# apache/incubator-predictionio

Measured on NVIDIA H100. Metric: ALS iterations/sec, higher is better.
Workload: dtype f32

## Files before the change

incubator-predictionio_b200/csrc/als_lockstep.cuh:

```cuda
#pragma once
#include <cuda_runtime.h>
#include <stdint.h>

namespace pio {

template <int N>
struct LsLayout {
  static constexpr int NBK = N / 16;
  static constexpr int NOFF = NBK * (NBK - 1) / 2;
  static constexpr int DIAG0 = NOFF * 256;
  static constexpr int SIZE = DIAG0 + NBK * 136;
  static constexpr int STRIDE = SIZE + ((SIZE % 32) == 16 ? 0 : (48 - SIZE % 32) % 32);
  __host__ __device__ static constexpr int swz(int rr) { return ((rr >> 1) & 1) * 2 + ((rr >> 2) & 1); }
  __host__ __device__ static constexpr int offd_base(int rb, int cb) { return (rb * (rb - 1) / 2 + cb) * 256; }
  __host__ __device__ static constexpr int offd(int rb, int cb, int rr, int cc) {
    return offd_base(rb, cb) + rr * 16 + 4 * ((cc >> 2) ^ swz(rr)) + (cc & 3);
  }
  __host__ __device__ static constexpr int diag(int rb, int rr, int cc) { return DIAG0 + rb * 136 + rr * (rr + 1) / 2 + cc; }
  __host__ __device__ static constexpr int at(int r, int c) {
    return (r >> 4) == (c >> 4) ? diag(r >> 4, r & 15, c & 15) : offd(r >> 4, c >> 4, r & 15, c & 15);
  }
};

__device__ __forceinline__ float ls_rsqrt(float x) {
  float r;
  asm("rsqrt.approx.ftz.f32 %0, %1;" : "=f"(r) : "f"(x));
  return r;
}

template <int N>
__device__ __forceinline__ void ls_add_yty(float* __restrict__ slot, const float* __restrict__ yty) {
  using LL = LsLayout<N>;
  const int lane = threadIdx.x & 31;
  for (int o = lane; o < LL::NOFF * 64; o += 32) {
    const int b = o >> 6, rr = (o >> 2) & 15, cg = o & 3;
    int rb = 1;
    while (rb * (rb + 1) / 2 <= b) ++rb;
    const int cb = b - rb * (rb - 1) / 2;
    float4* d = reinterpret_cast<float4*>(slot + LL::offd_base(rb, cb) + rr * 16 + 4 * (cg ^ LL::swz(rr)));
    const float4 y = __ldg(reinterpret_cast<const float4*>(yty + (size_t)(16 * rb + rr) * N + 16 * cb + 4 * cg));
    float4 v = *d;
    v.x += y.x; v.y += y.y; v.z += y.z; v.w += y.w;
    *d = v;
  }
  for (int o = lane; o < LL::NBK * 256; o += 32) {
    const int rb = o >> 8, rr = (o >> 4) & 15, cc = o & 15;
    if (cc <= rr) slot[LL::diag(rb, rr, cc)] += __ldg(yty + (size_t)(16 * rb + rr) * N + 16 * rb + cc);
  }
}

template <int N>
__device__ __forceinline__ void chol_lockstep(float* __restrict__ slot, const float* __restrict__ bvec, float ridge, int k,
                                              float* __restrict__ colbuf, float* __restrict__ dst_row, bool valid,
                                              int* __restrict__ fail) {
  using LL = LsLayout<N>;
  constexpr int LANES = N / 4;
  constexpr int Q = LANES / 16;
  constexpr int NBK = N / 16;
  static_assert(N == 64 || N == 128, "lockstep solver: N = 64 (two matrices per warp) or 128 (one)");
  const int lane = threadIdx.x & 31;
  const int l = lane % LANES, lq = l >> 4, lr = l & 15;
  const int sw = LL::swz(lr);
  float bb[4], yv[4], dv[4];
#pragma unroll
  for (int i = 0; i < 4; ++i) {
    bb[i] = bvec[i * LANES + l];
    yv[i] = 0.f;
    dv[i] = 0.f;
  }
  bool bad = false;
  __syncwarp();

#pragma unroll
  for (int p = 0; p < NBK; ++p) {
    constexpr int dummy = 0;
    (void)dummy;
    const int sp = p / Q;
    const bool isdiag = (Q == 1) || (lq == (p % Q));
    float a[4][16];
#pragma unroll
    for (int i = 0; i < 4; ++i) {
      if (i < sp) continue;
      const int bi = i * Q + lq;
      const int r = i * LANES + l;
      if (i == sp) {
#pragma unroll
        for (int c = 0; c < 16; ++c) {
          float v = 0.f;
          if (bi == p) {
            if (c <= lr) v = slot[LL::diag(p, lr, c)];
          } else if (bi > p) {
            v = slot[LL::offd(bi, p, lr, c)];
          }
          a[i][c] = v;
        }
      } else {
        const float* rowp = slot + LL::offd_base(bi, p) + lr * 16;
#pragma unroll
        for (int cg = 0; cg < 4; ++cg) {
          const float4 v = *reinterpret_cast<const float4*>(rowp + 4 * (cg ^ sw));
          a[i][4 * cg + 0] = v.x; a[i][4 * cg + 1] = v.y; a[i][4 * cg + 2] = v.z; a[i][4 * cg + 3] = v.w;
        }
      }
      if (i == sp) {
#pragma unroll
        for (int c = 0; c < 16; ++c)
          if (bi == p && c == lr) a[i][c] += ridge + (r >= k ? 1.f : 0.f);
      }
    }
    if (p > 0) {
#pragma unroll 1
      for (int q = 0; q < p; ++q) {
        const float* dblk = slot + LL::offd_base(p, q);
        const float* own[4];
#pragma unroll
        for (int i = 0; i < 4; ++i) {
          int bi = i * Q + lq;
          if (bi < p) bi = p;
          own[i] = slot + LL::offd_base(bi, q) + lr * 16;
        }
#pragma unroll 1
        for (int tg = 0; tg < 4; ++tg) {
          float4 o[4];
#pragma unroll
          for (int i = 0; i < 4; ++i)
            if (i >= sp) o[i] = *reinterpret_cast<const float4*>(own[i] + 4 * (tg ^ sw));
#pragma unroll
          for (int c = 0; c < 16; ++c) {
            const float4 d = *reinterpret_cast<const float4*>(dblk + c * 16 + 4 * (tg ^ LL::swz(c)));
#pragma unroll
            for (int i = 0; i < 4; ++i) {
              if (i < sp) continue;
              float v = a[i][c];
              v = fmaf(-o[i].x, d.x, v);
              v = fmaf(-o[i].y, d.y, v);
              v = fmaf(-o[i].z, d.z, v);
              v = fmaf(-o[i].w, d.w, v);
              a[i][c] = v;
            }
          }
        }
      }
    }
#pragma unroll
    for (int j = 0; j < 16; ++j) {
      float* cb = colbuf + (j & 1) * 32;
      if (isdiag) {
        cb[lr] = a[sp][j];
        cb[16 + lr] = bb[sp];
      }
      __syncwarp();
      float col[16];
#pragma unroll
      for (int cg = j / 4; cg < 4; ++cg) {
        const float4 v = *reinterpret_cast<const float4*>(cb + 4 * cg);
        col[4 * cg + 0] = v.x; col[4 * cg + 1] = v.y; col[4 * cg + 2] = v.z; col[4 * cg + 3] = v.w;
      }
      const float bg = cb[16 + j];
      float d = col[j];
      if (!(d > 0.f)) { bad = true; d = 1.f; }
      float inv = ls_rsqrt(d);
      inv = inv * (1.5f - 0.5f * d * inv * inv);
      const float inv2 = inv * inv;
      const float z = inv2 * bg;
      if (isdiag && lr == j) {
        yv[sp] = bg * inv;
        dv[sp] = inv;
      }
#pragma unroll
      for (int i = 0; i < 4; ++i) {
        if (i < sp) continue;
        const float aj = a[i][j];
        const float w = aj * inv2;
        if (i == sp) {
          const int bi = i * Q + lq;
          if (bi > p || (bi == p && lr > j)) bb[i] = fmaf(-aj, z, bb[i]);
        } else {
          bb[i] = fmaf(-aj, z, bb[i]);
        }
        a[i][j] = aj * inv;
#pragma unroll
        for (int c = j + 1; c < 16; ++c) a[i][c] = fmaf(-w, col[c], a[i][c]);
      }
    }
#pragma unroll
    for (int i = 0; i < 4; ++i) {
      if (i < sp) continue;
      const int bi = i * Q + lq;
      if (i == sp) {
#pragma unroll
        for (int c = 0; c < 16; ++c) {
          if (bi == p) {
            if (c <= lr) slot[LL::diag(p, lr, c)] = a[i][c];
          } else if (bi > p) {
            slot[LL::offd(bi, p, lr, c)] = a[i][c];
          }
        }
      } else {
        float* rowp = slot + LL::offd_base(bi, p) + lr * 16;
#pragma unroll
        for (int cg = 0; cg < 4; ++cg)
          *reinterpret_cast<float4*>(rowp + 4 * (cg ^ sw)) =
              make_float4(a[i][4 * cg + 0], a[i][4 * cg + 1], a[i][4 * cg + 2], a[i][4 * cg + 3]);
      }
    }
    __syncwarp();
  }

  float xs[4] = {0.f, 0.f, 0.f, 0.f};
#pragma unroll
  for (int g = N - 1; g >= 0; --g) {
    const int sg = g / LANES, lg = g % LANES, gb = g >> 4, gr = g & 15;
    const float t = yv[sg] * dv[sg];
    const float xg = __shfl_sync(0xffffffffu, t, lg, LANES);
    if (l == lg) xs[sg] = xg;
#pragma unroll
    for (int i = 0; i < 4; ++i) {
      if (i * Q > gb) continue;
      const int bi = i * Q + lq;
      if (bi < gb) yv[i] = fmaf(-slot[LL::offd(gb, bi, gr, lr)], xg, yv[i]);
      else if (bi == gb && lr < gr) yv[i] = fmaf(-slot[LL::diag(gb, gr, lr)], xg, yv[i]);
    }
  }
  if (valid) {
#pragma unroll
    for (int i = 0; i < 4; ++i) dst_row[i * LANES + l] = xs[i];
    if (bad && l == 0) atomicAdd(fail, 1);
  }
}

}
```

incubator-predictionio_b200/csrc/pio_als.cu:

```cuda
#include "../../include/pio_als.h"

#include <cuda_runtime.h>
#include <dlfcn.h>
#include <math.h>
#include <nccl.h>
#include <stdarg.h>
#include <stdio.h>
#include <stdlib.h>
#include <string.h>

#include <chrono>
#include <algorithm>
#include <array>
#include <deque>
#include <exception>
#include <map>
#include <mutex>
#include <string>
#include <type_traits>
#include <vector>

#include "als_kernels.cuh"
#include "als_mma_kernel.cuh"
#include "als_pair_kernel.cuh"
// ... 628 lines not shown
};
static int exchange_events(pio_als_handle* h, Scratch& keep, SortBufs& sb, long long n, XArr* arrs, int na,
                           long long* n_out) {
  cudaStream_t st = h->stream;
  NcclApi& nc = nccl_api();
  const int W = h->cfg.world_size, me = h->cfg.world_rank;
  Scratch tmp(h->stream);
  if (n > 0) CK(h, radix_sort_pairs(sb, (size_t)n, ceil_log2((uint64_t)W), st, &h->st.kernel_launches));
  const uint64_t* ks = sb.keys();
  const uint32_t* vs = sb.vals();
  long long *d_off = nullptr, *d_cnt = nullptr, *d_all = nullptr;
  CK(h, tmp.alloc(&d_off, (size_t)W + 1));
  CK(h, tmp.alloc(&d_cnt, (size_t)W));
  CK(h, tmp.alloc(&d_all, (size_t)W * W));
  CK(h, cudaMemsetAsync(d_off, 0, sizeof(long long) * (W + 1), st));
  if (n > 0) {
    build_ptr_kernel<<<nblk(n, 256), 256, 0, st>>>(ks, n, 0, W, d_off);
    LAUNCHED(h);
  }
  std::vector<long long> off(W + 1), all((size_t)W * W);
  CK(h, cudaMemcpyAsync(off.data(), d_off, sizeof(long long) * (W + 1), cudaMemcpyDeviceToHost, st));
  CK(h, cudaStreamSynchronize(st));
  std::vector<long long> cnt(W);
  for (int p = 0; p < W; ++p) cnt[p] = off[p + 1] - off[p];
  CK(h, cudaMemcpyAsync(d_cnt, cnt.data(), sizeof(long long) * W, cudaMemcpyHostToDevice, st));
  if (nc.AllGather(d_cnt, d_all, (size_t)W, ncclInt64, h->comm, st) != ncclSuccess)
    return fail(h, PIO_ALS_ERR_COMM, "ncclAllGather (exchange counts) failed");
  CK(h, cudaMemcpyAsync(all.data(), d_all, sizeof(long long) * W * W, cudaMemcpyDeviceToHost, st));
  CK(h, cudaStreamSynchronize(st));
  tmark(h, "  exchange: sort by rank + counts");
  std::vector<long long> roff(W + 1, 0);
  for (int src = 0; src < W; ++src) roff[src + 1] = roff[src] + all[(size_t)src * W + me];
  const long long nrecv = roff[W];
  if (nrecv >= (1ll << 32)) return fail(h, PIO_ALS_ERR_ARG, "more than 2^32-1 events on one rank after the exchange");
  std::vector<unsigned char*> sendbufs(na, nullptr), recvbufs(na, nullptr);
  for (int a = 0; a < na; ++a) {
    if (!arrs[a].in) { *arrs[a].out = nullptr; continue; }
    CK(h, tmp.alloc(&sendbufs[a], (size_t)(n > 0 ? n : 1) * arrs[a].elem));
    CK(h, keep.alloc(&recvbufs[a], (size_t)(nrecv > 0 ? nrecv : 1) * arrs[a].elem));
    if (n > 0) {
      if (arrs[a].elem == 4)
        gather_by_index_kernel<uint32_t><<<nblk(n, 256), 256, 0, st>>>((const uint32_t*)arrs[a].in, vs, n, (uint32_t*)sendbufs[a]);
      else
        gather_by_index_kernel<uint64_t><<<nblk(n, 256), 256, 0, st>>>((const uint64_t*)arrs[a].in, vs, n, (uint64_t*)sendbufs[a]);
      LAUNCHED(h);
    }
    *arrs[a].out = recvbufs[a];
  }
  if (nc.GroupStart() != ncclSuccess) return fail(h, PIO_ALS_ERR_COMM, "ncclGroupStart failed");
  for (int a = 0; a < na; ++a) {
    if (!arrs[a].in) continue;
    for (int p = 0; p < W; ++p) {
      const long long sc = cnt[p], rc_ = all[(size_t)p * W + me];
      if (sc > 0 && nc.Send(sendbufs[a] + (size_t)off[p] * arrs[a].elem, (size_t)sc * arrs[a].elem, ncclInt8, p, h->comm, st) != ncclSuccess)
        return fail(h, PIO_ALS_ERR_COMM, "ncclSend failed");
      if (rc_ > 0 && nc.Recv(recvbufs[a] + (size_t)roff[p] * arrs[a].elem, (size_t)rc_ * arrs[a].elem, ncclInt8, p, h->comm, st) != ncclSuccess)
        return fail(h, PIO_ALS_ERR_COMM, "ncclRecv failed");
    }
  }
  if (nc.GroupEnd() != ncclSuccess) return fail(h, PIO_ALS_ERR_COMM, "ncclGroupEnd failed");
  CK(h, cudaStreamSynchronize(st));
  tmark(h, "  exchange: gather + send/recv");
  *n_out = nrecv;
  return PIO_ALS_OK;
}

static int ingest_device(pio_als_handle* h, const int* d_user, const int* d_item, const float* d_rating,
                         long long nnz, int dedup, const long long* d_ts, bool sharded) {
  cudaStream_t st = h->stream;
  const int W = h->cfg.world_size;
  sharded = sharded && W > 1;
  if (nnz <= 0 && !sharded)
    return fail(h, PIO_ALS_ERR_ARG, "ratings cannot be empty (the templates require(!ratings.take(1).isEmpty))");
  if (nnz < 0) return fail(h, PIO_ALS_ERR_ARG, "nnz < 0");
  if (nnz >= (1ll << 32)) return fail(h, PIO_ALS_ERR_ARG, "nnz must be < 2^32 per call");
  if (dedup < 0 || dedup > 2) return fail(h, PIO_ALS_ERR_ARG, "bad dedup_mode %d", dedup);
  free_side(h, h->U, true);
  free_side(h, h->I, true);
  h->have_ratings = false;
  Side& U = h->U;
  Side& I = h->I;
  U.n = h->cfg.n_users;
  I.n = h->cfg.n_items;
  U.R = (U.n + W - 1) / W;
  I.R = (I.n + W - 1) / W;
  U.n_internal = U.R * W;
  I.n_internal = I.R * W;
  U.bits = ceil_log2((uint64_t)U.n_internal);
  I.bits = ceil_log2((uint64_t)I.n_internal);

  h->trace_on = getenv("PIO_ALS_INGEST_TRACE") != nullptr;
  h->t_prev = std::chrono::steady_clock::now();
  auto mark = [&](const char* what) { tmark(h, what); };
  CK(h, cudaMemsetAsync(h->d_fail, 0, sizeof(int), st));
  if (nnz > 0) {
    validate_coo_kernel<<<nblk(nnz, 256), 256, 0, st>>>(d_user, d_item, nnz, U.n, I.n, h->d_fail);
    LAUNCHED(h);
  }
  int bad = 0;
  CK(h, cudaMemcpyAsync(&bad, h->d_fail, sizeof(int), cudaMemcpyDeviceToHost, st));
  CK(h, cudaStreamSynchronize(st));
  if (bad) return fail(h, PIO_ALS_ERR_ARG, "%d ratings have a user/item index out of range", bad);

  mark("validate");
  Scratch tmp(h->stream);
  const int* su = d_user;
  const int* si = d_item;
  const float* sr = d_rating;
  const long long* sts = d_ts;
  long long ns = nnz;
  if (sharded && dedup != PIO_ALS_DEDUP_NONE) {
    Scratch xs(h->stream);
    SortBufs sb;
    for (int i : {0, 1}) {
      CK(h, xs.alloc(&sb.k[i], (size_t)nnz));
      CK(h, xs.alloc(&sb.v[i], (size_t)nnz));
    }
    if (nnz > 0) {
      dest_mod_kernel<<<nblk(nnz, 256), 256, 0, st>>>(d_user, nnz, W, sb.keys(), sb.vals());
      LAUNCHED(h);
    }
    void *xu = nullptr, *xi = nullptr, *xr = nullptr, *xt = nullptr;
    XArr arrs[4] = {{d_user, &xu, 4}, {d_item, &xi, 4}, {d_rating, &xr, 4},
                    {dedup == PIO_ALS_DEDUP_KEEP_LAST ? (const void*)d_ts : nullptr, &xt, 8}};
    int rc = exchange_events(h, tmp, sb, nnz, arrs, 4, &ns);
    if (rc) return rc;
    su = (const int*)xu; si = (const int*)xi; sr = (const float*)xr; sts = (const long long*)xt;
  }

  mark("exchange by user residue");
  const int* cu = su;
  const int* ci = si;
  const float* cr = sr;
  long long n2 = ns;
  if (dedup != PIO_ALS_DEDUP_NONE && ns > 0) {
    Scratch ds(h->stream);
    SortBufs sb;
    for (int i : {0, 1}) {
      CK(h, ds.alloc(&sb.k[i], (size_t)ns));
      CK(h, ds.alloc(&sb.v[i], (size_t)ns));
    }
    const int bu = ceil_log2((uint64_t)U.n), bi = ceil_log2((uint64_t)I.n);
    make_keys_ext_kernel<<<nblk(ns, 256), 256, 0, st>>>(su, si, ns, bi, sb.keys(), sb.vals());
    LAUNCHED(h);
    CK(h, radix_sort_pairs(sb, (size_t)ns, bu + bi, st, &h->st.kernel_launches));
    const uint64_t* ks = sb.keys();
    const uint32_t* vs = sb.vals();
    uint32_t* flag = nullptr;
    CK(h, ds.alloc(&flag, (size_t)ns));
    head_flags_kernel<<<nblk(ns, 256), 256, 0, st>>>(ks, ns, flag);
    LAUNCHED(h);
    uint32_t last_flag = 0, last_pos = 0;
    CK(h, cudaMemcpyAsync(&last_flag, flag + ns - 1, sizeof(uint32_t), cudaMemcpyDeviceToHost, st));
    CK(h, scan_exclusive_u32(flag, flag, (size_t)ns, st, &h->st.kernel_launches));
    CK(h, cudaMemcpyAsync(&last_pos, flag + ns - 1, sizeof(uint32_t), cudaMemcpyDeviceToHost, st));
    CK(h, cudaStreamSynchronize(st));
    n2 = (long long)last_pos + last_flag;
    int *du_ = nullptr, *di_ = nullptr;
    float* dr_ = nullptr;
    CK(h, tmp.alloc(&du_, (size_t)n2));
    CK(h, tmp.alloc(&di_, (size_t)n2));
    CK(h, tmp.alloc(&dr_, (size_t)n2));
    dedup_compact_kernel<<<nblk(ns, 256), 256, 0, st>>>(ks, vs, flag, ns, bi, sr, sts, dedup, du_, di_, dr_);
    LAUNCHED(h);
    cu = du_;
    ci = di_;
    cr = dr_;
  }

  mark("dedup");
  for (Side* s : {&U, &I}) {
    CK(h, dalloc(h, &s->deg, (size_t)s->n));
    CK(h, dalloc(h, &s->npos, (size_t)s->n));
    CK(h, dalloc(h, &s->perm, (size_t)s->n));
    CK(h, dalloc(h, &s->inv, (size_t)s->n_internal));
    CK(h, dalloc(h, &s->rpos, (size_t)s->n));
    CK(h, dalloc(h, &s->p2i, (size_t)s->n));
    CK(h, cudaMemsetAsync(s->deg, 0, sizeof(uint32_t) * s->n, st));
    CK(h, cudaMemsetAsync(s->npos, 0, sizeof(uint32_t) * s->n, st));
  }
  if (n2 > 0) {
    degree_kernel<<<nblk(n2, 256), 256, 0, st>>>(cu, ci, cr, n2, U.deg, I.deg, U.npos, I.npos);
    LAUNCHED(h);
  }
  CK(h, cudaMemsetAsync(h->d_absmax + 1, 0, sizeof(unsigned), st));
  if (n2 > 0) {
    pr::abs_max_kernel<<<std::min(nblk(n2, 256), 4u * h->sm_count), 256, 0, st>>>(cr, n2, h->d_absmax + 1);
    LAUNCHED(h);
  }
  long long n2_global = n2;
  if (sharded) {
    NcclApi& nc = nccl_api();
    long long* d_n = nullptr;
    CK(h, tmp.alloc(&d_n, 1));
    CK(h, cudaMemcpyAsync(d_n, &n2, sizeof(long long), cudaMemcpyHostToDevice, st));
    if (nc.GroupStart() != ncclSuccess) return fail(h, PIO_ALS_ERR_COMM, "ncclGroupStart failed");
    for (Side* s : {&U, &I}) {
      if (nc.AllReduce(s->deg, s->deg, (size_t)s->n, ncclUint32, ncclSum, h->comm, st) != ncclSuccess ||
          nc.AllReduce(s->npos, s->npos, (size_t)s->n, ncclUint32, ncclSum, h->comm, st) != ncclSuccess)
        return fail(h, PIO_ALS_ERR_COMM, "ncclAllReduce (degrees) failed");
    }
    if (nc.AllReduce(d_n, d_n, 1, ncclInt64, ncclSum, h->comm, st) != ncclSuccess ||
        nc.AllReduce(h->d_absmax + 1, h->d_absmax + 1, 1, ncclUint32, ncclMax, h->comm, st) != ncclSuccess)
      return fail(h, PIO_ALS_ERR_COMM, "ncclAllReduce (nnz, rating maximum) failed");
    if (nc.GroupEnd() != ncclSuccess) return fail(h, PIO_ALS_ERR_COMM, "ncclGroupEnd failed");
    CK(h, cudaMemcpyAsync(&n2_global, d_n, sizeof(long long), cudaMemcpyDeviceToHost, st));
    CK(h, cudaStreamSynchronize(st));
    if (n2_global <= 0)
      return fail(h, PIO_ALS_ERR_ARG, "ratings cannot be empty (the templates require(!ratings.take(1).isEmpty))");
  }
  h->st.nnz = n2_global;

  mark("degrees (+ all-reduce)");
  int rc = rank_rows(h, U);
  if (rc) return rc;
  rc = rank_rows(h, I);
  if (rc) return rc;

  mark("rank rows");
  if (!sharded) {
    rc = build_side(h, U, I, cu, ci, cr, n2, n2_global);
    if (rc) return rc;
    mark("build user side");
    rc = build_side(h, I, U, ci, cu, cr, n2, n2_global);
    if (rc) return rc;
    mark("build item side");
  } else {
    struct { Side* row; Side* col; const int* rowext; const int* colext; } jobs[2] = {{&U, &I, cu, ci}, {&I, &U, ci, cu}};
    for (auto& j : jobs) {
      Scratch xs(h->stream), recv(h->stream);
      SortBufs sb;
      for (int i : {0, 1}) {
        CK(h, xs.alloc(&sb.k[i], (size_t)n2));
        CK(h, xs.alloc(&sb.v[i], (size_t)n2));
      }
      if (n2 > 0) {
        dest_owner_kernel<<<nblk(n2, 256), 256, 0, st>>>(j.rowext, n2, j.row->perm, j.row->R, sb.keys(), sb.vals());
        LAUNCHED(h);
      }
      void *xrow = nullptr, *xcol = nullptr, *xr = nullptr;
      XArr arrs[3] = {{j.rowext, &xrow, 4}, {j.colext, &xcol, 4}, {cr, &xr, 4}};
      long long ne = 0;
      rc = exchange_events(h, recv, sb, n2, arrs, 3, &ne);
      if (rc) return rc;
      mark("exchange by row owner");
      rc = build_side(h, *j.row, *j.col, (const int*)xrow, (const int*)xcol, (const float*)xr, ne, n2_global);
      if (rc) return rc;
      mark("build side");
    }
  }

  for (Side* s : {&U, &I}) {
    if (!s->F) {
      CK(h, dalloc(h, &s->F, (size_t)s->n_internal * h->KP));
      h->have_init = false;
    }
    CK(h, dalloc(h, &s->cand_ext, (size_t)s->n_internal));
    cand_ext_kernel<<<nblk(s->n_internal, 256), 256, 0, st>>>(s->inv, s->deg, s->n_internal, s->cand_ext);
    LAUNCHED(h);
  }
  h->have_init = false;
  CK(h, cudaStreamSynchronize(st));
  mark("factor buffers");
  h->st.n_users_active = U.n_active;
  h->st.n_items_active = I.n_active;
  if (W > 1) {
    h->st.n_users_active = -1;
    h->st.n_items_active = -1;
  }
  h->have_ratings = true;
  h->trained = false;
  return PIO_ALS_OK;
}

static int init_hash(pio_als_handle* h) {
  cudaStream_t st = h->stream;
  CK(h, cudaMemsetAsync(h->U.F, 0, sizeof(float) * (size_t)h->U.n_internal * h->KP, st));
  CK(h, cudaMemsetAsync(h->I.F, 0, sizeof(float) * (size_t)h->I.n_internal * h->KP, st));
  hash_init_kernel<<<nblk(h->U.n, 128), 128, 0, st>>>(h->U.n, h->cfg.rank, h->KP, (uint64_t)h->cfg.seed, 0, h->U.perm,
                                                      h->U.deg, h->U.F);
  LAUNCHED(h);
  hash_init_kernel<<<nblk(h->I.n, 128), 128, 0, st>>>(h->I.n, h->cfg.rank, h->KP, (uint64_t)h->cfg.seed, 1, h->I.perm,
                                                      h->I.deg, h->I.F);
  LAUNCHED(h);
  h->have_init = true;
  return PIO_ALS_OK;
}

using Cfg16 = SolveCfg<16, 4, 25, 8>;
using Cfg32 = SolveCfg<32, 8, 25, 4>;
using Cfg64 = SolveCfg<64, 8, 7, 8>;
using Cfg128 = SolveCfg<128, 8, 2, 9>;

static_assert(fp32_rows_per_cta(16) == Cfg16::NG && fp32_rows_per_cta(32) == Cfg32::NG &&
              fp32_rows_per_cta(64) == Cfg64::NG && fp32_rows_per_cta(128) == Cfg128::NG, "SolveCfg::NG");
static_assert(Cfg16::WARP_CHOL && Cfg32::WARP_CHOL && Cfg64::WARP_CHOL && Cfg128::LS_PARTIAL,
              "als_finish_kernel runs one warp per row below KP 128, and KP 128 takes the LS128 route");
static_assert(MMA_ROWS_PER_CTA == mm::WARPS, "mm::WARPS");
static_assert(TC_ROWS_PER_CTA == tc::Api::kPerCta && TC_SOLVE_ROWS_PER_CTA == tc::Api::kSolveWarps, "tc::Api");
static_assert(LS128_FINISH_ROWS_PER_CTA == FIN128_WARPS, "FIN128_WARPS");
static_assert(PART % Cfg16::CH == 0 && PART % Cfg32::CH == 0 && PART % Cfg64::CH == 0 && PART % Cfg128::CH == 0 &&
              PART % mm::CH == 0 && PART % tc::STAGE_RATINGS == 0, "PART");
static_assert(PAIR_PART % pr::CH == 0 && pr::CH == 8, "PAIR_PART and PIO_ALS_PART round to multiples of pr::CH");

static int ensure_dyn_smem(pio_als_handle* h, const void* kernel, size_t bytes, bool carveout = false) {
  struct Rec {
    size_t bytes = 0;
    bool carveout = false;
  };
  static std::mutex mu;
  static std::map<std::pair<const void*, int>, Rec> recs;
  std::lock_guard<std::mutex> lk(mu);
  Rec& r = recs[std::make_pair(kernel, h->cfg.device)];
  if (r.bytes < bytes) {
    CK(h, cudaFuncSetAttribute(kernel, cudaFuncAttributeMaxDynamicSharedMemorySize, (int)bytes));
    r.bytes = bytes;
  }
  if (carveout && !r.carveout) {
    CK(h, cudaFuncSetAttribute(kernel, cudaFuncAttributePreferredSharedMemoryCarveout, 100));
    r.carveout = true;
  }
  return PIO_ALS_OK;
}

template <typename... KArgs, typename... Args>
static int solve_launch(pio_als_handle* h, void (*kernel)(KArgs...), int grid, int block, size_t smem, bool carveout,
                        cudaStream_t st, Args... args) {
  const int rc = ensure_dyn_smem(h, (const void*)kernel, smem, carveout);
  if (rc) return rc;
  kernel<<<grid, block, smem, st>>>(args...);
  LAUNCHED(h);
  ++h->st.solve_launches;
  CK(h, cudaGetLastError());
  return PIO_ALS_OK;
}

static void (*pair_kernel(int warps, bool imp))(const SolveParams, int) {
  switch (warps) {
    case 1: return imp ? pr::als_solve_pair_kernel<true, 1> : pr::als_solve_pair_kernel<false, 1>;
    case 2: return imp ? pr::als_solve_pair_kernel<true, 2> : pr::als_solve_pair_kernel<false, 2>;
    case 6: return imp ? pr::als_solve_pair_kernel<true, 6> : pr::als_solve_pair_kernel<false, 6>;
    case 12: return imp ? pr::als_solve_pair_kernel<true, 12> : pr::als_solve_pair_kernel<false, 12>;
    default: return imp ? pr::als_solve_pair_kernel<true, 4> : pr::als_solve_pair_kernel<false, 4>;
  }
}

static int tc_buffers(pio_als_handle* h, const Side& dst, tc::Api::Params* tp) {
  using A = tc::Api;
  tp->dbg = nullptr;
  tp->timing = nullptr;
  tp->out = nullptr;
  tp->out_row0 = 0;
  if (h->sw.tc_timing) {
    if (!h->d_timing) CK(h, cudaMalloc((void**)&h->d_timing, (size_t)h->sm_count * 16 * 8 * sizeof(long long)));
    cudaMemsetAsync(h->d_timing, 0, (size_t)h->sm_count * 16 * 8 * sizeof(long long), h->stream);
    tp->timing = h->d_timing;
  }
  if (h->sw.tc_debug) {
    if (h->dbg_rows < (size_t)dst.R) {
      if (h->d_dbg) cudaFree(h->d_dbg);
      CK(h, cudaMalloc((void**)&h->d_dbg, (size_t)dst.R * A::kRowFloats * sizeof(float)));
      h->dbg_rows = dst.R;
    }
    cudaMemsetAsync(h->d_dbg, 0, (size_t)dst.R * A::kRowFloats * sizeof(float), h->stream);
    tp->dbg = h->d_dbg;
  }
  if (h->sw.tc_split) {
    const int nlight = dst.n_active - dst.n_heavy;
    const size_t need = (size_t)(nlight < TC_TILE_ROWS ? nlight : TC_TILE_ROWS);
    if (h->tc_out_rows < need) {
      if (h->tc_out) cudaFree(h->tc_out);
      h->tc_out = nullptr;
      h->tc_out_rows = 0;
      CK(h, cudaMalloc((void**)&h->tc_out, need * A::kRowFloats * sizeof(float)));
      h->tc_out_rows = need;
    }
  }
  return PIO_ALS_OK;
}

template <class Cfg>
static int launch_solve_cfg(pio_als_handle* h, Side& dst, const Side& src) {
  SolveParams p0;
  p0.ptr = dst.ptr;
  p0.idx = dst.idx;
  p0.val = dst.val;
  p0.src = src.F;
  p0.dst = dst.F;
  p0.yty = h->yty;
  p0.nreg = dst.nreg;
  p0.fail = h->d_fail;
  p0.lambda = (float)h->cfg.lambda;
  p0.alpha = (float)h->cfg.alpha;
  p0.k = h->cfg.rank;
  p0.dst_row_offset = h->cfg.world_rank * dst.R;
  p0.absmax = h->d_absmax;
  p0.wl_beg = nullptr;
  p0.wl_end = nullptr;
  p0.partial = nullptr;
  p0.n_items = 0;
  const bool imp = h->cfg.implicit_prefs != 0;
  const SolvePlan plan = plan_half_step(h->sw, dst.plan, Cfg::KP, h->sm_count, dst.R, dst.n_active, dst.n_heavy,
                                        dst.n_parts, dst.h_row_part_ptr);
  const bool pair = dst.plan.kernel == SOLVE_PAIR;
  if (pair) cudaEventRecord(h->ev_start, h->stream);
  if (plan.partial_parts > 0 && !dst.partial) {
    const size_t floats = pair ? pr::PART_FLOATS : Cfg::PART_FLOATS;
    CK(h, cudaMallocAsync((void**)&dst.partial, sizeof(float) * (size_t)plan.partial_parts * floats, h->stream));
    if (pair) cudaEventRecord(h->ev_start, h->stream);
  }
  if (plan.n_aux > 0) cudaStreamWaitEvent(h->aux, h->ev_start, 0);
  size_t next_piece = 0;
  auto record_events = [&](int issued) {
    if (pair && issued == plan.n_aux) cudaEventRecord(h->ev_heavy, h->aux);
    for (; next_piece < plan.piece_after.size() && plan.piece_after[next_piece] == issued; ++next_piece)
      cudaEventRecord(h->ev_piece[next_piece], h->stream);
  };
  record_events(0);
  const int warps = h->sw.pair_warps;
  tc::Api::Params tp;
  bool tc_ready = false;
  for (size_t i = 0; i < plan.launches.size(); ++i) {
    const SolveLaunch& L = plan.launches[i];
    const cudaStream_t st = L.aux ? h->aux : h->stream;
    const int nrows = L.row_end - L.row_begin;
    SolveParams p = p0;
    if (L.stage == STAGE_ROWS || L.stage == STAGE_TC_SOLVE) {
      p.row_begin = L.row_begin;
      p.row_end = L.row_end;
    } else {
      p.wl_beg = dst.part_beg + L.wl_off;
      p.wl_end = dst.part_end + L.wl_off;
      p.partial = dst.partial;
      p.n_items = L.wl_count;
      p.row_begin = 0;
      p.row_end = dst.n_heavy;
    }
    auto fp32 = [&] {
      return solve_launch(h, imp ? als_solve_kernel<Cfg, true> : als_solve_kernel<Cfg, false>, L.grid, Cfg::NT,
                          Cfg::smem_bytes(), false, st, p);
    };
    auto pair_items = [&](int n_items) {
      return solve_launch(h, pair_kernel(warps, imp), L.grid, 32 * warps, pr::smem_bytes(warps), true, st, p, n_items);
    };
    int rc = PIO_ALS_OK;
    switch (L.stage) {
      case STAGE_PARTS:
        rc = pair ? pair_items(L.wl_count) : fp32();
        break;
      case STAGE_FINISH:
        rc = pair ? solve_launch(h, imp ? pr::als_finish_pair_kernel<true> : pr::als_finish_pair_kernel<false>, L.grid,
                                 32, pr::smem_bytes(1), true, st, p, dst.row_part_ptr, nrows)
                  : solve_launch(h, imp ? als_finish_kernel<Cfg, true> : als_finish_kernel<Cfg, false>, L.grid,
                                 32 * FINISH_ROWS_PER_CTA, sizeof(float) * 4 * (Cfg::SLOT + 4 * Cfg::KP), false, st, p,
                                 dst.row_part_ptr, nrows);
        break;
      case STAGE_LS128_TILE:
        rc = fp32();
        break;
      case STAGE_LS128_FINISH:
        rc = solve_launch(h, imp ? als_finish_ls128_kernel<true> : als_finish_ls128_kernel<false>, L.grid,
                          32 * FIN128_WARPS, sizeof(float) * (size_t)FIN128_FLOATS * FIN128_WARPS, false, st, p,
                          dst.row_part_ptr, L.row_begin, nrows, L.wl_off);
        break;
      case STAGE_ROWS:
        switch (dst.plan.kernel) {
          case SOLVE_PAIR:
            rc = pair_items(nrows);
            break;
          case SOLVE_MMA:
            rc = solve_launch(h, imp ? mm::als_solve_mma_kernel<true> : mm::als_solve_mma_kernel<false>, L.grid, mm::NT,
                              mm::SMEM_BYTES, false, st, p);
            break;
          case SOLVE_WGMMA:
            if (!tc_ready) {
              rc = tc_buffers(h, dst, &tp);
              if (rc) return rc;
              tc_ready = true;
            }
            tp.sp = p;
            tp.out = h->sw.tc_split ? h->tc_out : nullptr;
            tp.out_row0 = L.row_begin;
            rc = solve_launch(h, tc::Api::kernel(imp), L.grid, tc::Api::kThreads, tc::Api::kSmem, false, st, tp);
            break;
          default:
            rc = fp32();
        }
        break;
      case STAGE_TC_SOLVE:
        rc = solve_launch(h, tc::Api::solver(imp), L.grid, 32 * tc::Api::kSolveWarps, tc::Api::kSolveSmem, false, st, p,
                          (const float*)h->tc_out, L.row_begin);
        break;
    }
    if (rc) return rc;
    record_events((int)i + 1);
  }
  if (pair) {
    cudaStreamWaitEvent(h->stream, h->ev_heavy, 0);
    h->pieces_done = true;
  }
  return PIO_ALS_OK;
}

static int launch_solve(pio_als_handle* h, Side& dst, const Side& src) {
  switch (h->KP) {
    case 16: return launch_solve_cfg<Cfg16>(h, dst, src);
    case 32: return launch_solve_cfg<Cfg32>(h, dst, src);
    case 64: return launch_solve_cfg<Cfg64>(h, dst, src);
    default: return launch_solve_cfg<Cfg128>(h, dst, src);
  }
}

static bool gram_sharded(const pio_als_handle* h) { return h->cfg.world_size > 1 && GRAM_GROUPS % h->cfg.world_size == 0; }
static void gram_layout(const pio_als_handle* h, GramMap& m, int& my_groups, int& slot0) {
  const bool shard = gram_sharded(h);
  const int W = shard ? h->cfg.world_size : 1, me = shard ? h->cfg.world_rank : 0;
  my_groups = GRAM_GROUPS / W;
  slot0 = me * my_groups;
  int seen[GRAM_GROUPS] = {}, mine = 0;
  for (int g = 0; g < GRAM_GROUPS; ++g) {
    const int blk = g / W, pos = g % W;
    const int owner = (blk & 1) ? (W - 1 - pos) : pos;
    m.slot_of[g] = owner * my_groups + seen[owner]++;
    if (owner == me) m.cls[mine++] = g;
  }
  for (int lg = mine; lg < GRAM_GROUPS; ++lg) m.cls[lg] = 0;
}
static int gram_local(pio_als_handle* h, const Side& s) {
  GramMap m;
  int my_groups, slot0;
  gram_layout(h, m, my_groups, slot0);
  const int bpg = h->gram_blocks / GRAM_GROUPS, n = h->KP * h->KP, grid = my_groups * bpg;
  switch (h->KP) {
    case 16: gram_partial_kernel<16><<<grid, GRAM_THREADS, 0, h->stream>>>(s.F, s.p2i, s.n, h->gram_partial, slot0, bpg, m); break;
    case 32: gram_partial_kernel<32><<<grid, GRAM_THREADS, 0, h->stream>>>(s.F, s.p2i, s.n, h->gram_partial, slot0, bpg, m); break;
    case 64: gram_partial_kernel<64><<<grid, GRAM_THREADS, 0, h->stream>>>(s.F, s.p2i, s.n, h->gram_partial, slot0, bpg, m); break;
    default: gram_partial_kernel<128><<<grid, GRAM_THREADS, 0, h->stream>>>(s.F, s.p2i, s.n, h->gram_partial, slot0, bpg, m); break;
  }
  LAUNCHED(h);
  gram_group_kernel<<<dim3(nblk(n, 128), my_groups), 128, 0, h->stream>>>(h->gram_partial, bpg, n, slot0, h->gram_gsum);
  LAUNCHED(h);
  CK(h, cudaGetLastError());
  return PIO_ALS_OK;
}
static int gram_exchange(pio_als_handle* h, cudaStream_t comm_stream) {
  if (!gram_sharded(h)) return PIO_ALS_OK;
  const int n = h->KP * h->KP, my_groups = GRAM_GROUPS / h->cfg.world_size;
  const size_t cnt = (size_t)my_groups * n;
  if (nccl_api().AllGather(h->gram_gsum + (size_t)h->cfg.world_rank * cnt, h->gram_gsum, cnt, ncclDouble, h->comm, comm_stream) !=
      ncclSuccess)
    return fail(h, PIO_ALS_ERR_COMM, "ncclAllGather (YtY class sums) failed");
  return PIO_ALS_OK;
}
static int gram_reduce(pio_als_handle* h, const Side& s) {
  GramMap m;
  int my_groups, slot0;
  gram_layout(h, m, my_groups, slot0);
  const int n = h->KP * h->KP;
  gram_reduce_kernel<<<nblk(n, 256), 256, 0, h->stream>>>(h->gram_gsum, n, h->yty, m);
  LAUNCHED(h);
  CK(h, cudaGetLastError());
  h->gram_side = &s;
  return PIO_ALS_OK;
}

static int half_step(pio_als_handle* h, Side& dst, const Side& src, bool more) {
  cudaStream_t st = h->stream;
  const bool implicit = h->cfg.implicit_prefs != 0;
  if (implicit && h->gram_side != &src) {
    const EvPair e = next_ev(h, EV_GRAM);
    cudaEventRecord(e.a, st);
    int grc = gram_local(h, src);
    if (!grc) grc = gram_exchange(h, st);
    if (!grc) grc = gram_reduce(h, src);
    if (grc) return grc;
    cudaEventRecord(e.b, st);
  }
  {
    const EvPair e = next_ev(h, &dst == &h->U ? EV_SOLVE_USER : EV_SOLVE);
    cudaEventRecord(e.a, st);
    h->pieces_done = false;
    if (h->gram_side == &dst) h->gram_side = nullptr;
    if (dst.plan.kernel == SOLVE_PAIR) {
      const long long n = (long long)src.n_internal * h->KP;
      CK(h, cudaMemsetAsync(h->d_absmax, 0, sizeof(unsigned), st));
      pr::abs_max_kernel<<<4 * h->sm_count, 256, 0, st>>>(src.F, n, h->d_absmax);
      LAUNCHED(h);
    }
    const int rc = launch_solve(h, dst, src);
    if (rc) return rc;
    cudaEventRecord(e.b, st);
  }
  const bool prep = implicit && more;
  bool gram_pending = false;
  if (h->cfg.world_size > 1) {
    NcclApi& nc = nccl_api();
    const int W = h->cfg.world_size, me = h->cfg.world_rank;
    const EvPair e = next_ev(h, EV_COMM);
    if (h->pieces_done && h->sw.n_pieces > 1) {
      cudaStream_t sc = h->comm_st;
      const int C = h->sw.n_pieces;
      bool first = true;
      for (int c = 0; c < C; ++c) {
        const long long lo = (long long)dst.R * c / C, hi = (long long)dst.R * (c + 1) / C;
        if (hi <= lo) continue;
        cudaStreamWaitEvent(sc, h->ev_piece[c], 0);
// ... 3767 lines not shown
```

Measured before the change: 35.60.

## Use 3xTF32 tensor-core MMA for the N=64 lockstep Cholesky trailing update

```diff
diff --git a/incubator-predictionio_b200/csrc/als_lockstep.cuh b/incubator-predictionio_b200/csrc/als_lockstep.cuh
--- a/incubator-predictionio_b200/csrc/als_lockstep.cuh
+++ b/incubator-predictionio_b200/csrc/als_lockstep.cuh
@@ -26,6 +26,93 @@
   float r;
   asm("rsqrt.approx.ftz.f32 %0, %1;" : "=f"(r) : "f"(x));
   return r;
+}
+
+
+__device__ __forceinline__ void ls_split_tf32(float v, uint32_t& hi, uint32_t& lo) {
+  const uint32_t h = __float_as_uint(v) & 0xffffe000u;
+  const float r = __fsub_rn(v, __uint_as_float(h));
+  hi = h;
+  lo = (__float_as_uint(r) + 0x1000u) & 0xffffe000u;
+}
+__device__ __forceinline__ void ls_mma_tf32_z(float (&d)[4], const uint32_t (&a)[4], uint32_t b0, uint32_t b1) {
+  asm("mma.sync.aligned.m16n8k8.row.col.f32.tf32.tf32.f32 {%0,%1,%2,%3}, {%4,%5,%6,%7}, {%8,%9}, {%10,%10,%10,%10};\n"
+      : "=f"(d[0]), "=f"(d[1]), "=f"(d[2]), "=f"(d[3])
+      : "r"(a[0]), "r"(a[1]), "r"(a[2]), "r"(a[3]), "r"(b0), "r"(b1), "f"(0.f));
+}
+__device__ __forceinline__ void ls_mma_tf32(float (&d)[4], const uint32_t (&a)[4], uint32_t b0, uint32_t b1) {
+  asm("mma.sync.aligned.m16n8k8.row.col.f32.tf32.tf32.f32 {%0,%1,%2,%3}, {%4,%5,%6,%7}, {%8,%9}, {%0,%1,%2,%3};\n"
+      : "+f"(d[0]), "+f"(d[1]), "+f"(d[2]), "+f"(d[3])
+      : "r"(a[0]), "r"(a[1]), "r"(a[2]), "r"(a[3]), "r"(b0), "r"(b1));
+}
+
+template <int P>
+__device__ __forceinline__ void ls64_update_panel(float* __restrict__ slot) {
+  using LL = LsLayout<64>;
+  constexpr int NB = 4 - P;
+  const int lane = threadIdx.x & 31, g = lane >> 2, t = lane & 3;
+  const int sw = LL::swz(g);
+  float acc[NB][2][4];
+#pragma unroll
+  for (int nt = 0; nt < 2; ++nt) {
+    const int cc = 8 * nt + 2 * t;
+#pragma unroll
+    for (int e = 0; e < 2; ++e) {
+      acc[0][nt][e] = cc + e <= g ? slot[LL::diag(P, g, cc + e)] : 0.f;
+      acc[0][nt][2 + e] = cc + e <= g + 8 ? slot[LL::diag(P, g + 8, cc + e)] : 0.f;
+    }
+#pragma unroll
+    for (int ib = 1; ib < NB; ++ib) {
+      const float2 v0 = *reinterpret_cast<const float2*>(slot + LL::offd(P + ib, P, g, cc));
+      const float2 v1 = *reinterpret_cast<const float2*>(slot + LL::offd(P + ib, P, g + 8, cc));
+      acc[ib][nt][0] = v0.x; acc[ib][nt][1] = v0.y; acc[ib][nt][2] = v1.x; acc[ib][nt][3] = v1.y;
+    }
+  }
+  const int xo0 = g * 16 + t + 4 * (0 ^ sw), xo1 = g * 16 + t + 4 * (1 ^ sw);
+  const int xo2 = g * 16 + t + 4 * (2 ^ sw), xo3 = g * 16 + t + 4 * (3 ^ sw);
+#pragma unroll
+  for (int q = 0; q < P; ++q) {
+    uint32_t hi[NB][2][4], lo[NB][2][4];
+#pragma unroll
+    for (int ib = 0; ib < NB; ++ib) {
+      const float* bp = slot + LL::offd_base(P + ib, 0) + 256 * q;
+      const float v[2][4] = {{bp[xo0], bp[xo0 + 128], bp[xo1], bp[xo1 + 128]},
+                             {bp[xo2], bp[xo2 + 128], bp[xo3], bp[xo3 + 128]}};
+#pragma unroll
+      for (int ks = 0; ks < 2; ++ks)
+#pragma unroll
+        for (int r = 0; r < 4; ++r) ls_split_tf32(v[ks][r], hi[ib][ks][r], lo[ib][ks][r]);
+    }
+#pragma unroll
+    for (int ib = 0; ib < NB; ++ib) {
+#pragma unroll
+      for (int nt = 0; nt < 2; ++nt) {
+        float d[4];
+        ls_mma_tf32_z(d, lo[ib][0], hi[0][0][nt], hi[0][0][nt + 2]);
+        ls_mma_tf32(d, hi[ib][0], lo[0][0][nt], lo[0][0][nt + 2]);
+        ls_mma_tf32(d, hi[ib][0], hi[0][0][nt], hi[0][0][nt + 2]);
+        ls_mma_tf32(d, lo[ib][1], hi[0][1][nt], hi[0][1][nt + 2]);
+        ls_mma_tf32(d, hi[ib][1], lo[0][1][nt], lo[0][1][nt + 2]);
+        ls_mma_tf32(d, hi[ib][1], hi[0][1][nt], hi[0][1][nt + 2]);
+#pragma unroll
+        for (int e = 0; e < 4; ++e) acc[ib][nt][e] = __fsub_rn(acc[ib][nt][e], d[e]);
+      }
+    }
+  }
+#pragma unroll
+  for (int nt = 0; nt < 2; ++nt) {
+    const int cc = 8 * nt + 2 * t;
+#pragma unroll
+    for (int e = 0; e < 2; ++e) {
+      if (cc + e <= g) slot[LL::diag(P, g, cc + e)] = acc[0][nt][e];
+      if (cc + e <= g + 8) slot[LL::diag(P, g + 8, cc + e)] = acc[0][nt][2 + e];
+    }
+#pragma unroll
+    for (int ib = 1; ib < NB; ++ib) {
+      *reinterpret_cast<float2*>(slot + LL::offd(P + ib, P, g, cc)) = make_float2(acc[ib][nt][0], acc[ib][nt][1]);
+      *reinterpret_cast<float2*>(slot + LL::offd(P + ib, P, g + 8, cc)) = make_float2(acc[ib][nt][2], acc[ib][nt][3]);
+    }
+  }
 }
 
 template <int N>
@@ -77,6 +164,17 @@
     (void)dummy;
     const int sp = p / Q;
     const bool isdiag = (Q == 1) || (lq == (p % Q));
+    if (N == 64 && p > 0) {
+      float* s0 = slot - (lane >> 4) * LL::STRIDE;
+#pragma unroll 1
+      for (int m = 0; m < 2; ++m) {
+        float* sm = s0 + m * LL::STRIDE;
+        if (p == 1) ls64_update_panel<1>(sm);
+        else if (p == 2) ls64_update_panel<2>(sm);
+        else ls64_update_panel<3>(sm);
+      }
+      __syncwarp();
+    }
     float a[4][16];
 #pragma unroll
     for (int i = 0; i < 4; ++i) {
@@ -108,7 +206,7 @@
           if (bi == p && c == lr) a[i][c] += ridge + (r >= k ? 1.f : 0.f);
       }
     }
-    if (p > 0) {
+    if (N == 128 && p > 0) {
 #pragma unroll 1
       for (int q = 0; q < p; ++q) {
         const float* dblk = slot + LL::offd_base(p, q);
diff --git a/incubator-predictionio_b200/csrc/pio_als.cu b/incubator-predictionio_b200/csrc/pio_als.cu
--- a/incubator-predictionio_b200/csrc/pio_als.cu
+++ b/incubator-predictionio_b200/csrc/pio_als.cu
@@ -954,6 +954,7 @@
 static_assert(PART % Cfg16::CH == 0 && PART % Cfg32::CH == 0 && PART % Cfg64::CH == 0 && PART % Cfg128::CH == 0 &&
               PART % mm::CH == 0 && PART % tc::STAGE_RATINGS == 0, "PART");
 static_assert(PAIR_PART % pr::CH == 0 && pr::CH == 8, "PAIR_PART and PIO_ALS_PART round to multiples of pr::CH");
+static_assert(pr::SLOT_STRIDE == LsLayout<64>::STRIDE, "pair kernel slots: chol_lockstep<64> reads both");
 
 static int ensure_dyn_smem(pio_als_handle* h, const void* kernel, size_t bytes, bool carveout = false) {
   struct Rec {
```

Measured after the change: 36.18 (median of 6 runs). 1.02x the previous value.
